# KyanChen/RSPrompter

Hardware: NVIDIA H100
Metric: images/sec (higher is better)
Workload: dtype bf16

## Files before the change

rsprompter_b200/csrc/gemm.h:

```cpp
#pragma once
#include "host_util.h"

namespace rsp {

struct GemmArgs {
  const void* A = nullptr;
  const void* W = nullptr;
  void* out = nullptr;
  const float* bias = nullptr;
  const void* residual = nullptr;
  const int* row_map = nullptr;
  int M = 0, N = 0, K = 0;
  int lda = 0, ldw = 0, ldo = 0, ldr = 0;
  int res_mod = 0;
  int act = 0;
  int out_fp32 = 0;
  int res_fp32 = 1;
  int epi_mode = 0;
  const float* ln_gamma = nullptr;
  const float* ln_beta = nullptr;
  float ln_eps = 1e-6f;
  const int* res_block_map = nullptr;
  int res_block_rows = 0;
  const float* hyper = nullptr;
  float* mask_out = nullptr;
  int grid_h = 0, grid_w = 0;
  int conv_b = 0, conv_h = 0, conv_w = 0, conv_c = 0;
  int m_group_rows = 0, w_group_rows = 0;
};

int gemm_bf16(const GemmArgs& a, cudaStream_t stream);
int gemm_bf16_simt(const GemmArgs& a, cudaStream_t stream);
bool conv3x3_geometry_ok(int B, int H, int W, int C);
int conv3x3_bf16(const GemmArgs& a, cudaStream_t stream);
int gemm_upscale_masks(const GemmArgs& a, int n_out, cudaStream_t stream);

bool gemm_vector_rows(const GemmArgs& a);
int gemm_bf16_v2(const GemmArgs& a, cudaStream_t stream);
int gemm_bf16_v2_gelu_hyper_multi(const GemmArgs& a, int n_out, cudaStream_t stream);

}
```

rsprompter_b200/csrc/gemm_v2.cu:

```cuda
#include "gemm.h"
#include "sm90.cuh"

namespace rsp {

namespace v2 {

constexpr int BM = 128;
constexpr int BK = 64;
constexpr int A_BYTES = BM * BK * 2;
constexpr int STG_ROW = 136;
constexpr int STG_WARP = 32 * STG_ROW;
constexpr int BAR_BYTES = 256;
constexpr int SMEM_MAX = 227 * 1024;

enum { EPI_STD = 0, EPI_LN_ROW = 1, EPI_LN64_GELU = 2, EPI_GELU_HYPER = 3, EPI_GELU_HYPER2 = 4, EPI_GELU_HYPER3 = 5,
       EPI_LN_ROW_T = 6 };

__host__ __device__ constexpr int hyper_outputs(int epi) { return epi == EPI_GELU_HYPER3 ? 3 : epi == EPI_GELU_HYPER2 ? 2 : 1; }

template <int BN, int EPI>
struct Cfg {
  static constexpr bool SPLIT = EPI == EPI_STD;
  static_assert(!SPLIT || BN <= 128, "a 64 x 256 wgmma needs more registers than a 512-thread block has per thread");
  static constexpr int THREADS = SPLIT ? 512 : 384;
  static constexpr int EPI_WARPS = SPLIT ? 4 : 8;
  static constexpr int B_BYTES = BN * BK * 2;
  static constexpr int STAGE_BYTES = A_BYTES + B_BYTES;
  static constexpr int ACC_LD = BN + 4;
  static constexpr int ACC_BYTES = BM * ACC_LD * 4;
  static constexpr int ACC_BUFS = (SPLIT && BN <= 64) ? 2 : 1;
  static constexpr int STG_BYTES = EPI_WARPS * STG_WARP;
  static constexpr int STAGES = SPLIT ? ((BN == 128) ? 4 : (BN == 64) ? 5 : 8) : ((BN == 256) ? 1 : 3);
  static constexpr int SMEM_BYTES = STAGES * STAGE_BYTES + STG_BYTES + ACC_BUFS * ACC_BYTES + BAR_BYTES;
  static_assert(SMEM_BYTES <= SMEM_MAX, "shared memory");
  static_assert(2 * STAGES + 8 + 2 * ACC_BUFS <= BAR_BYTES / 8, "barrier area");
  static constexpr int NHALF = (!SPLIT && BN >= 128 && EPI != EPI_LN_ROW_T) ? 2 : 1;
  static constexpr int COLS_PER_WARP = BN / NHALF;
  static constexpr int REG_PRODUCER = 40;
  static constexpr int REG_MMA = 168;
  static constexpr int REG_EPI = 512 - REG_PRODUCER - 2 * REG_MMA;
  static_assert(REG_EPI >= 128 && REG_EPI % 8 == 0, "the epilogue warpgroup takes registers, never gives them up");
};

struct Dev {
  int M, N, K;
  const float* bias;
  const void* residual;
  void* out;
  const int* row_map;
  const int* res_block_map;
  int res_block_rows;
  int res_mod;
  int ldo, ldr;
  int act;
  int out_fp32;
  int res_fp32;
  int num_n_blocks;
  int num_tiles;
  const float* ln_gamma;
  const float* ln_beta;
  float ln_eps;
  const float* hyper;
  float* mask_out;
  int grid_h, grid_w;
  int conv_kb, conv_h, conv_w;
  int mblk_per_group, w_group_rows;
  int tma_store;
  int tma_res;
  int scalar_rows;
};

__device__ __forceinline__ int num_kblocks(const Dev& p) { return p.conv_kb > 0 ? 9 * p.conv_kb : (p.K + BK - 1) / BK; }

__device__ __forceinline__ int residual_row(const Dev& p, int orow) {
  if (p.res_block_map) {
    const int blk = orow / p.res_block_rows;
    return p.res_block_map[blk] * p.res_block_rows + (orow - blk * p.res_block_rows);
  }
  return p.res_mod > 0 ? (orow % p.res_mod) : orow;
}

__device__ __forceinline__ void add_bias_residual32(const Dev& p, float (&v)[32], int rrow, int col0) {
  if (p.bias) {
    const float4* b4 = reinterpret_cast<const float4*>(p.bias + col0);
#pragma unroll
    for (int i = 0; i < 8; ++i) {
      const float4 b = __ldg(b4 + i);
      v[4 * i + 0] += b.x; v[4 * i + 1] += b.y; v[4 * i + 2] += b.z; v[4 * i + 3] += b.w;
    }
  }
  if (p.residual) {
    if (p.res_fp32) {
      const float4* r4 = reinterpret_cast<const float4*>(
          static_cast<const float*>(p.residual) + static_cast<size_t>(rrow) * p.ldr + col0);
#pragma unroll
      for (int i = 0; i < 8; ++i) {
        const float4 x = r4[i];
        v[4 * i + 0] += x.x; v[4 * i + 1] += x.y; v[4 * i + 2] += x.z; v[4 * i + 3] += x.w;
      }
    } else {
      const uint4* r4 = reinterpret_cast<const uint4*>(
          static_cast<const __nv_bfloat16*>(p.residual) + static_cast<size_t>(rrow) * p.ldr + col0);
#pragma unroll
      for (int i = 0; i < 4; ++i) {
        const uint4 x = r4[i];
        const uint32_t w[4] = {x.x, x.y, x.z, x.w};
#pragma unroll
        for (int j = 0; j < 4; ++j) {
          const __nv_bfloat162 h = *reinterpret_cast<const __nv_bfloat162*>(&w[j]);
          v[8 * i + 2 * j + 0] += __bfloat162float(h.x);
          v[8 * i + 2 * j + 1] += __bfloat162float(h.y);
        }
      }
    }
  }
}

__device__ __forceinline__ void store32(const Dev& p, const float (&v)[32], int orow, int col0) {
  if (p.out_fp32) {
    float4* o4 = reinterpret_cast<float4*>(static_cast<float*>(p.out) + static_cast<size_t>(orow) * p.ldo + col0);
#pragma unroll
    for (int i = 0; i < 8; ++i) o4[i] = make_float4(v[4 * i + 0], v[4 * i + 1], v[4 * i + 2], v[4 * i + 3]);
  } else {
    uint4* o4 = reinterpret_cast<uint4*>(static_cast<__nv_bfloat16*>(p.out) + static_cast<size_t>(orow) * p.ldo + col0);
// ... 576 lines not shown
#pragma unroll
            for (int i = 0; i < 32; ++i) v[i] = fmaxf(v[i], 0.f);
          }
          if (stage_f32) {
            const uint32_t a = stg_s + lane * STG_ROW;
#pragma unroll
            for (int i = 0; i < 16; ++i)
              asm volatile("st.shared.v2.f32 [%0], {%1, %2};" ::"r"(a + i * 8), "f"(v[2 * i]), "f"(v[2 * i + 1])
                           : "memory");
          } else {
            const uint32_t a = stg_s + lane * STG_ROW + c * 64;
#pragma unroll
            for (int i = 0; i < 8; ++i)
              asm volatile("st.shared.v2.b32 [%0], {%1, %2};" ::"r"(a + i * 8),
                           "r"(pack_bf16x2(v[4 * i], v[4 * i + 1])), "r"(pack_bf16x2(v[4 * i + 2], v[4 * i + 3]))
                           : "memory");
          }
        }
        __syncwarp();
        const int col = col_pass + cl * epl;
        if (stage_f32) {
#pragma unroll
          for (int k = 0; k < 16; ++k) {
            const int rr = 2 * k + sub;
            const int orow = get_orow(rr);
            if (orow < 0 || col >= p.N) continue;
            float x0, x1;
            asm volatile("ld.shared.v2.f32 {%0, %1}, [%2];" : "=f"(x0), "=f"(x1) : "r"(stg_s + rr * STG_ROW + cl * 8));
            if (p.residual) {
              if (p.res_fp32 || p.scalar_rows) {
                x0 += resv[k].x; x1 += resv[k].y;
              } else {
                const uint32_t raw = __float_as_uint(resv[k].x);
                x0 += __uint_as_float(raw << 16); x1 += __uint_as_float(raw & 0xffff0000u);
              }
            }
            if (p.scalar_rows) {
              store_at(p, orow, col, x0);
              if (col + 1 < p.N) store_at(p, orow, col + 1, x1);
            } else if (p.out_fp32)
              *reinterpret_cast<float2*>(static_cast<float*>(p.out) + static_cast<size_t>(orow) * p.ldo + col) =
                  make_float2(x0, x1);
            else
              *reinterpret_cast<uint32_t*>(static_cast<__nv_bfloat16*>(p.out) + static_cast<size_t>(orow) * p.ldo +
                                           col) = pack_bf16x2(x0, x1);
          }
        } else {
#pragma unroll 4
          for (int r0 = 0; r0 < 32; r0 += rpi) {
            const int rr = r0 + sub;
            const int orow = get_orow(rr);
            if (orow < 0 || col >= p.N) continue;
            uint32_t w0, w1;
            asm volatile("ld.shared.v2.b32 {%0, %1}, [%2];" : "=r"(w0), "=r"(w1) : "r"(stg_s + rr * STG_ROW + cl * 8));
            *reinterpret_cast<uint2*>(static_cast<__nv_bfloat16*>(p.out) + static_cast<size_t>(orow) * p.ldo + col) =
                make_uint2(w0, w1);
          }
        }
        __syncwarp();
      }
    }
  }
}

template <int BN, int EPI, int OUT>
__device__ __forceinline__ void epilogue_loop(const Dev& p, const CUtensorMap& tma_c, const CUtensorMap& tma_r, int e,
                                              uint32_t acc_base, uint8_t* stg_all, uint64_t* bar_res,
                                              uint64_t* bar_tfull, uint64_t* bar_tempty) {
  using C = Cfg<BN, EPI>;
  uint32_t rphase = 0;
  for (int tile = blockIdx.x; tile < p.num_tiles; tile += gridDim.x) {
    const int m_blk = tile / p.num_n_blocks;
    const int n_blk = tile % p.num_n_blocks;
    const int it = (tile - blockIdx.x) / gridDim.x;
    const int buf = C::ACC_BUFS == 2 ? (it & 1) : 0;
    const uint32_t use = C::ACC_BUFS == 2 ? (it >> 1) : it;
    mbar_wait(smem_u32(&bar_tfull[buf]), use & 1);
    epilogue_tile<BN, EPI, OUT>(p, tma_c, tma_r, m_blk, n_blk, e, 0, acc_base + buf * C::ACC_BYTES, stg_all, bar_res,
                                rphase);
    mbar_arrive(smem_u32(&bar_tempty[buf]));
  }
}

template <int BN, int EPI>
__global__ void __launch_bounds__(Cfg<BN, EPI>::THREADS, 1)
gemm_bf16_wgmma_v2_kernel(const __grid_constant__ CUtensorMap tma_a, const __grid_constant__ CUtensorMap tma_b,
                            const __grid_constant__ CUtensorMap tma_c, const __grid_constant__ CUtensorMap tma_r,
                            const Dev p) {
  using C = Cfg<BN, EPI>;
  constexpr int STAGES = C::STAGES;
  extern __shared__ __align__(1024) uint8_t smem[];
  const uint32_t smem_base = smem_u32(smem);
  uint8_t* stg_all = smem + STAGES * C::STAGE_BYTES;
  const uint32_t acc_base = smem_u32(stg_all + C::STG_BYTES);
  uint64_t* bars = reinterpret_cast<uint64_t*>(stg_all + C::STG_BYTES + C::ACC_BUFS * C::ACC_BYTES);
  uint64_t* bar_full = bars;
  uint64_t* bar_empty = bars + STAGES;
  uint64_t* bar_res = bars + 2 * STAGES;
  uint64_t* bar_tfull = bar_res + 8;
  uint64_t* bar_tempty = bar_tfull + C::ACC_BUFS;

  const int warp = threadIdx.x >> 5;
  const int lane = threadIdx.x & 31;

  if (threadIdx.x == 0) {
    tma_prefetch_desc(&tma_a);
    tma_prefetch_desc(&tma_b);
    for (int s = 0; s < STAGES; ++s) {
      mbar_init(smem_u32(&bar_full[s]), 1);
      mbar_init(smem_u32(&bar_empty[s]), 8);
    }
    for (int s = 0; s < 8; ++s) mbar_init(smem_u32(&bar_res[s]), 1);
    for (int b = 0; b < C::ACC_BUFS; ++b) {
      mbar_init(smem_u32(&bar_tfull[b]), 256);
      mbar_init(smem_u32(&bar_tempty[b]), 32 * C::EPI_WARPS);
    }
    fence_barrier_init();
  }
  __syncthreads();

  if (warp < 4) {
    if constexpr (C::SPLIT) setmaxnreg_dec<C::REG_PRODUCER>();
    if (warp == 0 && lane == 0) {
      const int num_kb = num_kblocks(p);
      int stage = 0;
      uint32_t phase = 0;
      for (int tile = blockIdx.x; tile < p.num_tiles; tile += gridDim.x) {
        const int m_blk = tile / p.num_n_blocks;
        const int n_blk = tile % p.num_n_blocks;
        int cb = 0, cy = 0, cx = 0, tap = 0, ckb = 0;
        const int w_row0 = p.mblk_per_group > 0 ? (m_blk / p.mblk_per_group) * p.w_group_rows : 0;
        if (p.conv_kb > 0) {
          const int hw = p.conv_h * p.conv_w, p0 = m_blk * BM;
          cb = p0 / hw;
          const int rem = p0 - cb * hw;
          cy = rem / p.conv_w;
          cx = rem - cy * p.conv_w;
        }
        for (int kb = 0; kb < num_kb; ++kb) {
          mbar_wait(smem_u32(&bar_empty[stage]), phase ^ 1);
          const uint32_t full = smem_u32(&bar_full[stage]);
          const uint32_t sa = smem_base + stage * C::STAGE_BYTES;
          mbar_expect_tx(full, C::STAGE_BYTES);
          if (p.conv_kb > 0) {
            const int ky = tap / 3, kx = tap - 3 * ky;
            tma_load_4d(sa, &tma_a, full, ckb * BK, cx + kx - 1, cy + ky - 1, cb);
            if (++ckb == p.conv_kb) { ckb = 0; ++tap; }
          } else {
            tma_load_2d(sa, &tma_a, full, kb * BK, m_blk * BM);
          }
          tma_load_2d(sa + A_BYTES, &tma_b, full, kb * BK, n_blk * BN + w_row0);
          if (++stage == STAGES) { stage = 0; phase ^= 1; }
        }
      }
      for (int i = 0; i < STAGES; ++i) {
        mbar_wait(smem_u32(&bar_empty[stage]), phase ^ 1);
        if (++stage == STAGES) { stage = 0; phase ^= 1; }
      }
    }
  } else if (warp < 12) {
    if constexpr (C::SPLIT) setmaxnreg_inc<C::REG_MMA>();
    const int wg = (warp - 4) >> 2;
    const int num_kb = num_kblocks(p);
    int kstage = 0;
    uint32_t kphase = 0;
    if constexpr (C::SPLIT) {
      int it = 0;
      for (int tile = blockIdx.x; tile < p.num_tiles; tile += gridDim.x, ++it) {
        float acc[BN / 2];
        wg_mainloop<BN, STAGES>(acc, smem_base, C::STAGE_BYTES, A_BYTES, num_kb, wg, kstage, kphase, bar_full,
                                bar_empty);
        const int buf = C::ACC_BUFS == 2 ? (it & 1) : 0;
        const uint32_t use = C::ACC_BUFS == 2 ? (it >> 1) : it;
        mbar_wait(smem_u32(&bar_tempty[buf]), (use & 1) ^ 1);
        acc_store<BN>(acc, acc_base + buf * C::ACC_BYTES, C::ACC_LD, wg, threadIdx.x & 127);
        mbar_arrive(smem_u32(&bar_tfull[buf]));
      }
    } else {
      const int e = warp - 4;
      uint32_t rphase = 0;
      for (int tile = blockIdx.x; tile < p.num_tiles; tile += gridDim.x) {
        const int m_blk = tile / p.num_n_blocks;
        const int n_blk = tile % p.num_n_blocks;
        {
          float acc[BN / 2];
          wg_mainloop<BN, STAGES>(acc, smem_base, C::STAGE_BYTES, A_BYTES, num_kb, wg, kstage, kphase, bar_full,
                                  bar_empty);
          named_bar_sync(5, 256);
          acc_store<BN>(acc, acc_base, C::ACC_LD, wg, threadIdx.x & 127);
          named_bar_sync(5, 256);
        }
        if (wg < C::NHALF)
          epilogue_tile<BN, EPI>(p, tma_c, tma_r, m_blk, n_blk, e, wg, acc_base, stg_all, bar_res, rphase);
      }
      if (p.tma_store && lane == 0) bulk_wait0();
    }
  } else if constexpr (C::SPLIT) {
    setmaxnreg_inc<C::REG_EPI>();
    const int e = warp - 12;
    if (p.tma_store) {
      epilogue_loop<BN, EPI, OUT_TMA>(p, tma_c, tma_r, e, acc_base, stg_all, bar_res, bar_tfull, bar_tempty);
      if (lane == 0) bulk_wait0();
    } else {
      epilogue_loop<BN, EPI, OUT_SCATTER>(p, tma_c, tma_r, e, acc_base, stg_all, bar_res, bar_tfull, bar_tempty);
    }
  }
}

template <int BN, int EPI>
static int launch(const GemmArgs& a, cudaStream_t stream) {
  using C = Cfg<BN, EPI>;
  CUtensorMap ta, tb;
  Dev p;
  p.conv_kb = 0; p.conv_h = a.conv_h; p.conv_w = a.conv_w;
  if (a.conv_c > 0) {
    const uint64_t C_ = a.conv_c, W_ = a.conv_w, H_ = a.conv_h, B_ = a.conv_b;
    const uint32_t tw = a.conv_w < BM ? a.conv_w : BM;
    const uint32_t th = (BM / tw) < static_cast<uint32_t>(a.conv_h) ? BM / tw : a.conv_h;
    const uint32_t tb = BM / (tw * th);
    uint64_t dims[4] = {C_, W_, H_, B_};
    uint64_t strides[3] = {C_ * 2, W_ * C_ * 2, H_ * W_ * C_ * 2};
    uint32_t box[4] = {static_cast<uint32_t>(BK), tw, th, tb};
    RSP_TRY(make_tmap_bf16(&ta, a.A, 4, dims, strides, box));
    p.conv_kb = a.conv_c / BK;
  } else {
    RSP_TRY(make_tmap_bf16_2d(&ta, a.A, a.M, a.K, static_cast<uint64_t>(a.lda) * 2, BM, BK));
  }
  const int n_groups = a.m_group_rows > 0 ? (a.M + a.m_group_rows - 1) / a.m_group_rows : 1;
  const uint64_t w_rows = a.m_group_rows > 0 ? static_cast<uint64_t>(n_groups - 1) * a.w_group_rows + a.N : a.N;
  RSP_TRY(make_tmap_bf16_2d(&tb, a.W, w_rows, a.K, static_cast<uint64_t>(a.ldw) * 2, BN, BK));
  CUtensorMap tc = tb, tr = tb;
  p.tma_store = 0;
  p.tma_res = 0;
  p.scalar_rows = EPI == EPI_STD && !gemm_vector_rows(a);
  {
    const uint64_t esz = a.out_fp32 ? 4 : 2;
    bool res_ok = true;
    if (a.residual) {
      res_ok = (a.res_fp32 != 0) == (a.out_fp32 != 0) &&
               (reinterpret_cast<uintptr_t>(a.residual) & 15) == 0 && (static_cast<uint64_t>(a.ldr) * esz) % 16 == 0 &&
               (a.res_block_map ? (a.res_block_rows % 32 == 0 && a.M % 32 == 0) : (a.res_mod == 0 || a.res_mod % 32 == 0));
    }
    if ((EPI == EPI_STD || EPI == EPI_LN_ROW || EPI == EPI_LN64_GELU) && BN >= 64 && res_ok && !a.row_map &&
        !p.scalar_rows && a.out &&
        (reinterpret_cast<uintptr_t>(a.out) & 15) == 0 && (static_cast<uint64_t>(a.ldo) * esz) % 16 == 0) {
      uint64_t dims[2] = {static_cast<uint64_t>(a.N), static_cast<uint64_t>(a.M)};
      uint64_t strides[1] = {static_cast<uint64_t>(a.ldo) * esz};
      uint32_t box[2] = {a.out_fp32 ? 32u : 64u, 32u};
      RSP_TRY(make_tmap(&tc, a.out, 2, dims, strides, box, a.out_fp32));
      p.tma_store = 1;
      if (a.residual) {
        const uint64_t rrows = a.res_block_map ? (1ull << 31) : (a.res_mod > 0 ? a.res_mod : a.M);
        uint64_t rdims[2] = {static_cast<uint64_t>(a.N), rrows};
        uint64_t rstrides[1] = {static_cast<uint64_t>(a.ldr) * esz};
        RSP_TRY(make_tmap(&tr, a.residual, 2, rdims, rstrides, box, a.out_fp32));
        p.tma_res = 1;
      }
    }
  }
  if (EPI == EPI_LN_ROW && !(p.tma_store && p.tma_res)) {
    set_last_error("gemm_v2: fused row LayerNorm needs TMA-eligible bf16 output and residual");
    return RSP_ERR_INVALID;
  }
  p.M = a.M; p.N = a.N; p.K = a.K;
  p.bias = a.bias; p.residual = a.residual; p.out = a.out; p.row_map = a.row_map;
  p.res_block_map = a.res_block_map; p.res_block_rows = a.res_block_rows;
  p.res_mod = a.res_mod; p.ldo = a.ldo; p.ldr = a.ldr; p.act = a.act;
  p.out_fp32 = a.out_fp32; p.res_fp32 = a.res_fp32;
  p.mblk_per_group = a.m_group_rows > 0 ? a.m_group_rows / BM : 0;
  p.w_group_rows = a.w_group_rows;
  p.num_n_blocks = (a.N + BN - 1) / BN;
  p.num_tiles = ((a.M + BM - 1) / BM) * p.num_n_blocks;
  p.ln_gamma = a.ln_gamma; p.ln_beta = a.ln_beta; p.ln_eps = a.ln_eps;
  p.hyper = a.hyper; p.mask_out = a.mask_out; p.grid_h = a.grid_h; p.grid_w = a.grid_w;
  auto kern = gemm_bf16_wgmma_v2_kernel<BN, EPI>;
  static bool attr_set_dev[kMaxDevices] = {};
  bool& attr_set = attr_set_dev[current_device()];
  if (!attr_set) {
    RSP_CHECK_CUDA(cudaFuncSetAttribute(kern, cudaFuncAttributeMaxDynamicSharedMemorySize, C::SMEM_BYTES));
    attr_set = true;
  }
  const int grid = p.num_tiles < num_sms() ? p.num_tiles : num_sms();
  kern<<<grid, C::THREADS, C::SMEM_BYTES, stream>>>(ta, tb, tc, tr, p);
  RSP_CHECK_LAUNCH();
  return RSP_OK;
}

}

bool gemm_vector_rows(const GemmArgs& a) {
  const bool stage_f32 = a.out_fp32 || a.residual;
  const uintptr_t po = reinterpret_cast<uintptr_t>(a.out), pr = reinterpret_cast<uintptr_t>(a.residual);
  if (stage_f32) {
    if (a.N % 2 != 0 || a.ldo % 2 != 0 || (po & (a.out_fp32 ? 7 : 3)) != 0) return false;
  } else {
    if (a.N % 4 != 0 || a.ldo % 4 != 0 || (po & 7) != 0) return false;
  }
  if (a.residual && (a.ldr % 2 != 0 || (pr & (a.res_fp32 ? 7 : 3)) != 0)) return false;
  if (a.bias && (reinterpret_cast<uintptr_t>(a.bias) & 15) != 0) return false;
  return true;
}

static bool ln_row_tma(const GemmArgs& a) {
  return a.N == 256 && !a.out_fp32 && a.residual && !a.res_fp32 && a.bias && a.res_mod == 0 && a.act == 0 &&
         (a.res_block_map ? (a.res_block_rows % 32 == 0 && a.M % 32 == 0) : true);
}

int gemm_bf16_v2(const GemmArgs& a, cudaStream_t stream) {
  if (a.epi_mode == v2::EPI_STD) {
    if (a.N > 64) return v2::launch<128, v2::EPI_STD>(a, stream);
    if (a.N > 32) return v2::launch<64, v2::EPI_STD>(a, stream);
    return v2::launch<32, v2::EPI_STD>(a, stream);
  }
  if (a.epi_mode == v2::EPI_LN_ROW) {
    if (ln_row_tma(a)) return v2::launch<256, v2::EPI_LN_ROW>(a, stream);
    return a.N > 128 ? v2::launch<256, v2::EPI_LN_ROW_T>(a, stream) : v2::launch<128, v2::EPI_LN_ROW_T>(a, stream);
  }
  if (a.epi_mode == v2::EPI_LN64_GELU) return v2::launch<128, v2::EPI_LN64_GELU>(a, stream);
  return v2::launch<128, v2::EPI_GELU_HYPER>(a, stream);
}

int gemm_bf16_v2_gelu_hyper_multi(const GemmArgs& a, int n_out, cudaStream_t stream) {
  switch (n_out) {
    case 1: return v2::launch<128, v2::EPI_GELU_HYPER>(a, stream);
    case 2: return v2::launch<128, v2::EPI_GELU_HYPER2>(a, stream);
    case 3: return v2::launch<128, v2::EPI_GELU_HYPER3>(a, stream);
    default: set_last_error("gemm_v2: %d hypernetwork outputs (1 to 3)", n_out); return RSP_ERR_INVALID;
  }
}

}
```

rsprompter_b200/csrc/selftest.cu:

```cuda
#include <math.h>
#include <stdio.h>
#include <stdlib.h>
#include <string.h>

#include <vector>

#include "gemm.h"
#include "sm90.cuh"

namespace rsp { const char* last_error(); }
using namespace rsp;

#define CK(x)                                                                      \
  do {                                                                             \
    cudaError_t e = (x);                                                           \
    if (e != cudaSuccess) {                                                        \
      printf("CUDA error %s at %s:%d\n", cudaGetErrorString(e), __FILE__, __LINE__); \
      exit(2);                                                                     \
    }                                                                              \
  } while (0)

static uint32_t g_seed = 12345;
static float frand() {
  g_seed = g_seed * 1664525u + 1013904223u;
// ... 64 lines not shown
  a.out = dO1;
  int s = gemm_bf16(a, 0);
  if (s) { printf("[%s] gemm_bf16 failed: %s\n", c.name, last_error()); return 1; }
  cudaError_t e = cudaDeviceSynchronize();
  if (e != cudaSuccess) { printf("[%s] kernel error: %s\n", c.name, cudaGetErrorString(e)); exit(3); }
  a.out = dO2;
  s = gemm_bf16_simt(a, 0);
  if (s) { printf("[%s] simt failed: %s\n", c.name, last_error()); return 1; }
  CK(cudaDeviceSynchronize());
  std::vector<uint8_t> h1(osz), h2(osz);
  CK(cudaMemcpy(h1.data(), dO1, osz, cudaMemcpyDeviceToHost));
  CK(cudaMemcpy(h2.data(), dO2, osz, cudaMemcpyDeviceToHost));
  double maxerr = 0, maxref = 0;
  size_t nbad = 0;
  const size_t n = (size_t)out_rows * N;
  for (size_t i = 0; i < n; ++i) {
    float x, y;
    if (c.out_fp32) { x = ((float*)h1.data())[i]; y = ((float*)h2.data())[i]; }
    else {
      uint32_t ux = (uint32_t)((uint16_t*)h1.data())[i] << 16, uy = (uint32_t)((uint16_t*)h2.data())[i] << 16;
      memcpy(&x, &ux, 4); memcpy(&y, &uy, 4);
    }
    const double d = fabs((double)x - (double)y);
    if (!(d <= 1e-2 * (1.0 + fabs(y)))) ++nbad;
    if (d > maxerr || d != d) maxerr = d;
    if (fabs(y) > maxref) maxref = fabs(y);
  }
  printf("[%s] M=%d N=%d K=%d  max|diff|=%.3e  max|ref|=%.3e  bad=%zu/%zu  %s\n", c.name, M, N, K,
         maxerr, maxref, nbad, n, nbad == 0 ? "PASS" : "FAIL");
  if (nbad) {
    for (int r = 0; r < 4 && r < out_rows; ++r) {
      printf("   row %d:", r);
      for (int j = 0; j < 8 && j < N; ++j) {
        float x, y;
        size_t i = (size_t)r * N + j;
        if (c.out_fp32) { x = ((float*)h1.data())[i]; y = ((float*)h2.data())[i]; }
        else {
          uint32_t ux = (uint32_t)((uint16_t*)h1.data())[i] << 16, uy = (uint32_t)((uint16_t*)h2.data())[i] << 16;
          memcpy(&x, &ux, 4); memcpy(&y, &uy, 4);
        }
        printf(" %.3f/%.3f", x, y);
      }
      printf("\n");
    }
  }
  cudaFree(dA); cudaFree(dW); cudaFree(db); cudaFree(dO1); cudaFree(dO2); cudaFree(dres);
  if (dmap) cudaFree(dmap);
  return nbad ? 1 : 0;
}

static void bench_gemm(int M, int N, int K, int act, int out_fp32, int residual, int res_bf16 = 0, int iters = 20, int res_mod = 0) {
  void *dA, *dW, *dO, *dR = nullptr;
  float* db;
  CK(cudaMalloc(&dA, (size_t)M * K * 2));
  CK(cudaMalloc(&dW, (size_t)N * K * 2));
  CK(cudaMalloc(&dO, (size_t)M * N * 4));
  CK(cudaMalloc(&db, N * 4));
  CK(cudaMemset(dA, 0x11, (size_t)M * K * 2));
  CK(cudaMemset(dW, 0x11, (size_t)N * K * 2));
  CK(cudaMemset(db, 0, N * 4));
  if (residual) { CK(cudaMalloc(&dR, (size_t)M * N * 4)); CK(cudaMemset(dR, 0, (size_t)M * N * 4)); }
  (void)res_bf16;
  GemmArgs a;
  a.A = dA; a.W = dW; a.out = dO; a.bias = db; a.M = M; a.N = N; a.K = K;
  a.lda = K; a.ldw = K; a.ldo = N; a.ldr = N; a.act = act; a.out_fp32 = out_fp32;
  a.residual = dR; a.res_fp32 = res_bf16 ? 0 : 1; a.res_mod = res_mod;
  for (int i = 0; i < 3; ++i) gemm_bf16(a, 0);
  CK(cudaDeviceSynchronize());
  cudaEvent_t e0, e1;
  cudaEventCreate(&e0); cudaEventCreate(&e1);
  cudaEventRecord(e0);
  for (int i = 0; i < iters; ++i) gemm_bf16(a, 0);
  cudaEventRecord(e1);
  CK(cudaDeviceSynchronize());
  float ms;
  cudaEventElapsedTime(&ms, e0, e1);
  ms /= iters;
  const double bytes = (double)M * K * 2 + (double)N * K * 2 + (double)M * N * (out_fp32 ? 4 : 2) +
                       (residual ? (double)M * N * (res_bf16 ? 2 : 4) : 0.0);
  printf("bench gemm M=%d N=%d K=%d act=%d outf32=%d res=%d%s: %.3f ms  %.1f TFLOP/s  %.0f GB/s\n", M, N, K,
         act, out_fp32, residual, res_bf16 ? "(bf16)" : "", ms, 2.0 * M * N * K / ms * 1e-9, bytes / ms * 1e-6);
  cudaFree(dA); cudaFree(dW); cudaFree(dO); cudaFree(db);
  if (dR) cudaFree(dR);
}

int selftest_attention(int bench);


int main(int argc, char** argv) {
  const char* what = argc > 1 ? argv[1] : "all";
  const int bench = argc > 2 && !strcmp(argv[2], "bench");
  int fails = 0;
  cudaDeviceProp prop;
  CK(cudaGetDeviceProperties(&prop, 0));
  printf("device: %s sm_%d%d, %d SMs\n", prop.name, prop.major, prop.minor, prop.multiProcessorCount);
  if (!strcmp(what, "gemm") || !strcmp(what, "all")) {
    const Case cases[] = {
        {"tiny-f32",            128,  128,   64,  0, 0, 0, 1, 1, 0, 0},
        {"k128-f32",            256,  256,  128,  0, 0, 0, 1, 1, 0, 0},
        {"n512-f32",            384,  512,  256,  1, 0, 0, 1, 1, 0, 0},
        {"bn64",                200,   64,  192,  1, 2, 0, 1, 0, 0, 0},
        {"bn32",                200,   32,  192,  1, 2, 0, 1, 0, 0, 0},
        {"ragged-n",            300,   40,  128,  1, 0, 0, 1, 1, 0, 0},
        {"bias-gelu-bf16",     1000,  768,  768,  1, 1, 0, 1, 0, 0, 0},
        {"resid-f32",          1000,  768, 3072,  1, 0, 1, 1, 1, 0, 0},
        {"resid-bf16",          777,  256,  320,  1, 2, 1, 0, 0, 0, 0},
        {"rowmap-resid",       4000, 2304,  768,  1, 0, 1, 1, 1, 1, 0},
        {"posembed-mod",       2048,  768,  768,  1, 0, 1, 1, 1, 0, 512},
        {"multi-tile-per-cta", 40000, 256,  128,  1, 0, 0, 1, 0, 0, 0},
    };
    for (const Case& c : cases) fails += run_case(c);
    if (bench) {
      bench_gemm(39200, 3840, 1280, 0, 0, 0);
      bench_gemm(32768, 1280, 1280, 0, 1, 1);
      bench_gemm(32768, 5120, 1280, 1, 0, 0);
      bench_gemm(32768, 1280, 5120, 0, 1, 1);
      bench_gemm(32768, 768, 3072, 0, 1, 1);
      bench_gemm(8192, 8192, 8192, 0, 0, 0);
    }
  }
  if (!strcmp(what, "gemmprof")) {
    bench_gemm(1 << 20, 256, 128, 0, 1, 1, 1, 3);
    bench_gemm(1 << 20, 128, 256, 0, 0, 0, 0, 3);
    bench_gemm(1 << 20, 256, 128, 0, 0, 0, 0, 3);
    bench_gemm(1 << 20, 128, 256, 0, 0, 1, 0, 3, 4096);
  }
  if (!strcmp(what, "attn") || !strcmp(what, "all")) fails += selftest_attention(bench);
  printf("selftest: %d failing case(s)\n", fails);
  return fails ? 1 : 0;
}
```

rsprompter_b200/csrc/sm90.cuh:

```cuda
#pragma once
#include <cuda.h>
#include <cuda_bf16.h>
#include <cuda_runtime.h>
#include <stdint.h>

namespace rsp {

__device__ __forceinline__ uint32_t smem_u32(const void* p) {
  return static_cast<uint32_t>(__cvta_generic_to_shared(p));
}

__device__ __forceinline__ uint32_t elect_one() {
  uint32_t pred = 0;
  asm volatile(
      "{\n"
      ".reg .b32 rx;\n"
      ".reg .pred px;\n"
      "elect.sync rx|px, 0xffffffff;\n"
      "selp.u32 %0, 1, 0, px;\n"
      "}\n"
      : "=r"(pred));
  return pred;
}

__device__ __forceinline__ void mbar_init(uint32_t bar, uint32_t count) {
  asm volatile("mbarrier.init.shared::cta.b64 [%0], %1;" ::"r"(bar), "r"(count) : "memory");
}
__device__ __forceinline__ void fence_barrier_init() {
  asm volatile("fence.mbarrier_init.release.cluster;" ::: "memory");
}
__device__ __forceinline__ void fence_proxy_async_smem() {
  asm volatile("fence.proxy.async.shared::cta;" ::: "memory");
}
__device__ __forceinline__ void mbar_expect_tx(uint32_t bar, uint32_t bytes) {
  asm volatile("mbarrier.arrive.expect_tx.shared::cta.b64 _, [%0], %1;" ::"r"(bar), "r"(bytes)
               : "memory");
}
__device__ __forceinline__ void mbar_arrive(uint32_t bar) {
  asm volatile("mbarrier.arrive.shared::cta.b64 _, [%0];" ::"r"(bar) : "memory");
}
__device__ __forceinline__ uint32_t mbar_try_wait(uint32_t bar, uint32_t parity) {
  uint32_t ok;
  asm volatile(
      "{\n"
      ".reg .pred p;\n"
      "mbarrier.try_wait.parity.shared::cta.b64 p, [%1], %2;\n"
      "selp.u32 %0, 1, 0, p;\n"
      "}\n"
      : "=r"(ok)
      : "r"(bar), "r"(parity)
      : "memory");
  return ok;
}
__device__ __forceinline__ void mbar_wait(uint32_t bar, uint32_t parity) {
  if (mbar_try_wait(bar, parity)) return;
  long long t0 = clock64();
  uint32_t spins = 0;
  while (!mbar_try_wait(bar, parity)) {
    if ((++spins & 0x3ff) == 0 && clock64() - t0 > (1ll << 31)) __trap();
  }
}

__device__ __forceinline__ void tma_prefetch_desc(const CUtensorMap* m) {
  asm volatile("prefetch.tensormap [%0];" ::"l"(m) : "memory");
}
__device__ __forceinline__ void tma_load_2d(uint32_t dst, const CUtensorMap* m, uint32_t bar,
                                            int c0, int c1) {
  asm volatile(
      "cp.async.bulk.tensor.2d.shared::cluster.global.mbarrier::complete_tx::bytes"
      " [%0], [%1, {%3, %4}], [%2];" ::"r"(dst),
      "l"(m), "r"(bar), "r"(c0), "r"(c1)
      : "memory");
}
__device__ __forceinline__ void tma_load_3d(uint32_t dst, const CUtensorMap* m, uint32_t bar,
                                            int c0, int c1, int c2) {
  asm volatile(
      "cp.async.bulk.tensor.3d.shared::cluster.global.mbarrier::complete_tx::bytes"
      " [%0], [%1, {%3, %4, %5}], [%2];" ::"r"(dst),
      "l"(m), "r"(bar), "r"(c0), "r"(c1), "r"(c2)
      : "memory");
}
__device__ __forceinline__ void tma_load_4d(uint32_t dst, const CUtensorMap* m, uint32_t bar,
                                            int c0, int c1, int c2, int c3) {
  asm volatile(
      "cp.async.bulk.tensor.4d.shared::cluster.global.mbarrier::complete_tx::bytes"
      " [%0], [%1, {%3, %4, %5, %6}], [%2];" ::"r"(dst),
      "l"(m), "r"(bar), "r"(c0), "r"(c1), "r"(c2), "r"(c3)
      : "memory");
}

__device__ __forceinline__ void tma_store_2d(const CUtensorMap* m, uint32_t src, int c0, int c1) {
  asm volatile("cp.async.bulk.tensor.2d.global.shared::cta.bulk_group [%0, {%2, %3}], [%1];" ::"l"(m), "r"(src),
               "r"(c0), "r"(c1)
               : "memory");
}
__device__ __forceinline__ void bulk_commit() { asm volatile("cp.async.bulk.commit_group;" ::: "memory"); }
__device__ __forceinline__ void bulk_wait_read0() { asm volatile("cp.async.bulk.wait_group.read 0;" ::: "memory"); }
__device__ __forceinline__ void bulk_wait0() { asm volatile("cp.async.bulk.wait_group 0;" ::: "memory"); }

__device__ __forceinline__ uint64_t make_gdesc(uint32_t saddr, uint32_t lbo_bytes, uint32_t sbo_bytes) {
  uint64_t d = 0;
  d |= static_cast<uint64_t>((saddr & 0x3ffff) >> 4);
  d |= static_cast<uint64_t>((lbo_bytes >> 4) & 0x3fff) << 16;
  d |= static_cast<uint64_t>((sbo_bytes >> 4) & 0x3fff) << 32;
  d |= 1ull << 62;
  return d;
}

__device__ __forceinline__ uint64_t make_gdesc_sw32(uint32_t saddr, uint32_t lbo_bytes, uint32_t sbo_bytes) {
  uint64_t d = 0;
  d |= static_cast<uint64_t>((saddr & 0x3ffff) >> 4);
  d |= static_cast<uint64_t>((lbo_bytes >> 4) & 0x3fff) << 16;
  d |= static_cast<uint64_t>((sbo_bytes >> 4) & 0x3fff) << 32;
  d |= 3ull << 62;
  return d;
}

__device__ __forceinline__ void wgmma_fence() { asm volatile("wgmma.fence.sync.aligned;" ::: "memory"); }
__device__ __forceinline__ void wgmma_commit() { asm volatile("wgmma.commit_group.sync.aligned;" ::: "memory"); }
template <int N>
__device__ __forceinline__ void wgmma_wait() { asm volatile("wgmma.wait_group.sync.aligned %0;" ::"n"(N) : "memory"); }
template <int R>
__device__ __forceinline__ void acc_fence(float (&d)[R]) {
#pragma unroll
  for (int i = 0; i < R; ++i) asm volatile("" : "+f"(d[i])::"memory");
}

template <int N>
struct Wgmma;
template <> struct Wgmma<32> {
  template <int TB>
  __device__ __forceinline__ static void ss(float (&d)[16], uint64_t a, uint64_t b, uint32_t acc) {
    asm volatile(
        "{\n.reg .pred p;\n"
        "setp.ne.b32 p, %18, 0;\n"
        "wgmma.mma_async.sync.aligned.m64n32k16.f32.bf16.bf16 "
        "{" 
        "%0, %1, %2, %3, %4, %5, %6, %7, %8, %9, %10, %11, %12, %13, %14, %15"
        "}, %16, %17, p, 1, 1, 0, %19;\n}\n"
        : "+f"(d[0]), "+f"(d[1]), "+f"(d[2]), "+f"(d[3]), "+f"(d[4]), "+f"(d[5]), "+f"(d[6]), "+f"(d[7]),
          "+f"(d[8]), "+f"(d[9]), "+f"(d[10]), "+f"(d[11]), "+f"(d[12]), "+f"(d[13]), "+f"(d[14]), "+f"(d[15])
        : "l"(a), "l"(b), "r"(acc), "n"(TB));
  }
};
template <> struct Wgmma<64> {
  template <int TB>
  __device__ __forceinline__ static void ss(float (&d)[32], uint64_t a, uint64_t b, uint32_t acc) {
    asm volatile(
        "{\n.reg .pred p;\n"
        "setp.ne.b32 p, %34, 0;\n"
        "wgmma.mma_async.sync.aligned.m64n64k16.f32.bf16.bf16 "
        "{" 
        "%0, %1, %2, %3, %4, %5, %6, %7, %8, %9, %10, %11, %12, %13, %14, %15, "
        "%16, %17, %18, %19, %20, %21, %22, %23, %24, %25, %26, %27, %28, %29, %30, %31"
        "}, %32, %33, p, 1, 1, 0, %35;\n}\n"
        : "+f"(d[0]), "+f"(d[1]), "+f"(d[2]), "+f"(d[3]), "+f"(d[4]), "+f"(d[5]), "+f"(d[6]), "+f"(d[7]),
          "+f"(d[8]), "+f"(d[9]), "+f"(d[10]), "+f"(d[11]), "+f"(d[12]), "+f"(d[13]), "+f"(d[14]), "+f"(d[15]),
          "+f"(d[16]), "+f"(d[17]), "+f"(d[18]), "+f"(d[19]), "+f"(d[20]), "+f"(d[21]), "+f"(d[22]), "+f"(d[23]),
          "+f"(d[24]), "+f"(d[25]), "+f"(d[26]), "+f"(d[27]), "+f"(d[28]), "+f"(d[29]), "+f"(d[30]), "+f"(d[31])
        : "l"(a), "l"(b), "r"(acc), "n"(TB));
  }
};
template <> struct Wgmma<128> {
  template <int TB>
  __device__ __forceinline__ static void ss(float (&d)[64], uint64_t a, uint64_t b, uint32_t acc) {
    asm volatile(
        "{\n.reg .pred p;\n"
        "setp.ne.b32 p, %66, 0;\n"
        "wgmma.mma_async.sync.aligned.m64n128k16.f32.bf16.bf16 "
        "{" 
        "%0, %1, %2, %3, %4, %5, %6, %7, %8, %9, %10, %11, %12, %13, %14, %15, "
        "%16, %17, %18, %19, %20, %21, %22, %23, %24, %25, %26, %27, %28, %29, %30, %31, "
        "%32, %33, %34, %35, %36, %37, %38, %39, %40, %41, %42, %43, %44, %45, %46, %47, "
        "%48, %49, %50, %51, %52, %53, %54, %55, %56, %57, %58, %59, %60, %61, %62, %63"
        "}, %64, %65, p, 1, 1, 0, %67;\n}\n"
        : "+f"(d[0]), "+f"(d[1]), "+f"(d[2]), "+f"(d[3]), "+f"(d[4]), "+f"(d[5]), "+f"(d[6]), "+f"(d[7]),
          "+f"(d[8]), "+f"(d[9]), "+f"(d[10]), "+f"(d[11]), "+f"(d[12]), "+f"(d[13]), "+f"(d[14]), "+f"(d[15]),
          "+f"(d[16]), "+f"(d[17]), "+f"(d[18]), "+f"(d[19]), "+f"(d[20]), "+f"(d[21]), "+f"(d[22]), "+f"(d[23]),
          "+f"(d[24]), "+f"(d[25]), "+f"(d[26]), "+f"(d[27]), "+f"(d[28]), "+f"(d[29]), "+f"(d[30]), "+f"(d[31]),
          "+f"(d[32]), "+f"(d[33]), "+f"(d[34]), "+f"(d[35]), "+f"(d[36]), "+f"(d[37]), "+f"(d[38]), "+f"(d[39]),
// ... 211 lines not shown
```

Before: 61.16.

## Add 128x256 wide GEMM schedule with register epilogue for large plain GEMMs

Adds a new EPI_STD_WIDE kernel variant that uses 128x256 tiles. The two MMA warpgroups hold 232 registers each and run the epilogue straight from registers, writing swizzled bf16 slabs to shared memory and storing them with double-buffered TMA stores. This drops the separate epilogue warpgroup and the fp32 shared-memory accumulator staging. The variant is selected automatically for plain bias/activation GEMMs with N divisible by 256, K >= 1024 and enough tiles. This raises per-tile arithmetic intensity but serialises the epilogue with the mainloop for each tile, so there is no overlap. A/B benchmarks and a correctness case are added to the selftest.

New measurement: 63.07 (median of 6 runs). 1.03x the previous value.

```diff
diff --git a/rsprompter_b200/csrc/gemm.h b/rsprompter_b200/csrc/gemm.h
--- a/rsprompter_b200/csrc/gemm.h
+++ b/rsprompter_b200/csrc/gemm.h
@@ -37,6 +37,7 @@
 
 bool gemm_vector_rows(const GemmArgs& a);
 int gemm_bf16_v2(const GemmArgs& a, cudaStream_t stream);
+int gemm_bf16_v2_std(const GemmArgs& a, bool wide, cudaStream_t stream);
 int gemm_bf16_v2_gelu_hyper_multi(const GemmArgs& a, int n_out, cudaStream_t stream);
 
 }
diff --git a/rsprompter_b200/csrc/gemm_v2.cu b/rsprompter_b200/csrc/gemm_v2.cu
--- a/rsprompter_b200/csrc/gemm_v2.cu
+++ b/rsprompter_b200/csrc/gemm_v2.cu
@@ -14,7 +14,7 @@
 constexpr int SMEM_MAX = 227 * 1024;
 
 enum { EPI_STD = 0, EPI_LN_ROW = 1, EPI_LN64_GELU = 2, EPI_GELU_HYPER = 3, EPI_GELU_HYPER2 = 4, EPI_GELU_HYPER3 = 5,
-       EPI_LN_ROW_T = 6 };
+       EPI_LN_ROW_T = 6, EPI_STD_WIDE = 7 };
 
 __host__ __device__ constexpr int hyper_outputs(int epi) { return epi == EPI_GELU_HYPER3 ? 3 : epi == EPI_GELU_HYPER2 ? 2 : 1; }
 
@@ -22,24 +22,28 @@
 struct Cfg {
   static constexpr bool SPLIT = EPI == EPI_STD;
   static_assert(!SPLIT || BN <= 128, "a 64 x 256 wgmma needs more registers than a 512-thread block has per thread");
+  static constexpr bool WIDE = EPI == EPI_STD_WIDE;
+  static_assert(!WIDE || BN == 256, "the register epilogue is written for the 64 x 256 fragment");
   static constexpr int THREADS = SPLIT ? 512 : 384;
   static constexpr int EPI_WARPS = SPLIT ? 4 : 8;
   static constexpr int B_BYTES = BN * BK * 2;
   static constexpr int STAGE_BYTES = A_BYTES + B_BYTES;
   static constexpr int ACC_LD = BN + 4;
   static constexpr int ACC_BYTES = BM * ACC_LD * 4;
-  static constexpr int ACC_BUFS = (SPLIT && BN <= 64) ? 2 : 1;
+  static constexpr int ACC_BUFS = WIDE ? 0 : (SPLIT && BN <= 64) ? 2 : 1;
   static constexpr int STG_BYTES = EPI_WARPS * STG_WARP;
-  static constexpr int STAGES = SPLIT ? ((BN == 128) ? 4 : (BN == 64) ? 5 : 8) : ((BN == 256) ? 1 : 3);
+  static constexpr int STAGES =
+      WIDE ? 4 : SPLIT ? ((BN == 128) ? 4 : (BN == 64) ? 5 : 8) : ((BN == 256) ? 1 : 3);
   static constexpr int SMEM_BYTES = STAGES * STAGE_BYTES + STG_BYTES + ACC_BUFS * ACC_BYTES + BAR_BYTES;
   static_assert(SMEM_BYTES <= SMEM_MAX, "shared memory");
   static_assert(2 * STAGES + 8 + 2 * ACC_BUFS <= BAR_BYTES / 8, "barrier area");
   static constexpr int NHALF = (!SPLIT && BN >= 128 && EPI != EPI_LN_ROW_T) ? 2 : 1;
   static constexpr int COLS_PER_WARP = BN / NHALF;
   static constexpr int REG_PRODUCER = 40;
-  static constexpr int REG_MMA = 168;
-  static constexpr int REG_EPI = 512 - REG_PRODUCER - 2 * REG_MMA;
-  static_assert(REG_EPI >= 128 && REG_EPI % 8 == 0, "the epilogue warpgroup takes registers, never gives them up");
+  static constexpr int REG_MMA = WIDE ? 232 : 168;
+  static_assert(!WIDE || REG_PRODUCER + 2 * REG_MMA <= 3 * 168, "wide schedule register budget");
+  static constexpr int REG_EPI = SPLIT ? 512 - REG_PRODUCER - 2 * REG_MMA : 0;
+  static_assert(!SPLIT || (REG_EPI >= 128 && REG_EPI % 8 == 0), "the epilogue warpgroup takes registers, never gives them up");
 };
 
 struct Dev {
@@ -782,6 +786,44 @@
   }
 }
 
+__device__ __forceinline__ void epilogue_wide(const Dev& p, const CUtensorMap& tma_c, const float (&acc)[128],
+                                              int m_blk, int n_blk, int wg, int e, uint8_t* stg_all) {
+  const int lane = threadIdx.x & 31;
+  const int r = lane >> 2;
+  const int row0 = m_blk * BM + wg * 64 + (e & 3) * 16;
+  const uint32_t slab = smem_u32(stg_all) + e * 4096;
+  const float* bias = p.bias;
+  const int act = p.act;
+#pragma unroll
+  for (int s = 0; s < 4; ++s) {
+    const int col0 = n_blk * 256 + s * 64;
+    const uint32_t half = slab + (s & 1) * 2048;
+    if (lane == 0) bulk_wait_read1();
+    __syncwarp();
+#pragma unroll
+    for (int c = 0; c < 8; ++c) {
+      float v[4] = {acc[32 * s + 4 * c], acc[32 * s + 4 * c + 1], acc[32 * s + 4 * c + 2], acc[32 * s + 4 * c + 3]};
+      if (bias) {
+        const float2 b = __ldg(reinterpret_cast<const float2*>(bias + col0 + 8 * c + 2 * (lane & 3)));
+        v[0] += b.x; v[1] += b.y; v[2] += b.x; v[3] += b.y;
+      }
+      if (act == 1) {
+#pragma unroll
+        for (int i = 0; i < 4; ++i) v[i] = gelu_fast(v[i]);
+      } else if (act == 2) {
+#pragma unroll
+        for (int i = 0; i < 4; ++i) v[i] = fmaxf(v[i], 0.f);
+      }
+      const uint32_t a = half + r * 128 + ((c ^ r) << 4) + 4 * (lane & 3);
+      asm volatile("st.shared.b32 [%0], %1;" ::"r"(a), "r"(pack_bf16x2(v[0], v[1])) : "memory");
+      asm volatile("st.shared.b32 [%0], %1;" ::"r"(a + 8 * 128), "r"(pack_bf16x2(v[2], v[3])) : "memory");
+    }
+    fence_proxy_async_smem();
+    __syncwarp();
+    if (lane == 0) { tma_store_2d(&tma_c, half, col0, row0); bulk_commit(); }
+  }
+}
+
 template <int BN, int EPI>
 __global__ void __launch_bounds__(Cfg<BN, EPI>::THREADS, 1)
 gemm_bf16_wgmma_v2_kernel(const __grid_constant__ CUtensorMap tma_a, const __grid_constant__ CUtensorMap tma_b,
@@ -820,7 +862,7 @@
   __syncthreads();
 
   if (warp < 4) {
-    if constexpr (C::SPLIT) setmaxnreg_dec<C::REG_PRODUCER>();
+    if constexpr (C::SPLIT || C::WIDE) setmaxnreg_dec<C::REG_PRODUCER>();
     if (warp == 0 && lane == 0) {
       const int num_kb = num_kblocks(p);
       int stage = 0;
@@ -859,12 +901,20 @@
       }
     }
   } else if (warp < 12) {
-    if constexpr (C::SPLIT) setmaxnreg_inc<C::REG_MMA>();
+    if constexpr (C::SPLIT || C::WIDE) setmaxnreg_inc<C::REG_MMA>();
     const int wg = (warp - 4) >> 2;
     const int num_kb = num_kblocks(p);
     int kstage = 0;
     uint32_t kphase = 0;
-    if constexpr (C::SPLIT) {
+    if constexpr (C::WIDE) {
+      for (int tile = blockIdx.x; tile < p.num_tiles; tile += gridDim.x) {
+        float acc[BN / 2];
+        wg_mainloop<BN, STAGES>(acc, smem_base, C::STAGE_BYTES, A_BYTES, num_kb, wg, kstage, kphase, bar_full,
+                                bar_empty);
+        epilogue_wide(p, tma_c, acc, tile / p.num_n_blocks, tile % p.num_n_blocks, wg, warp - 4, stg_all);
+      }
+      if (lane == 0) bulk_wait0();
+    } else if constexpr (C::SPLIT) {
       int it = 0;
       for (int tile = blockIdx.x; tile < p.num_tiles; tile += gridDim.x, ++it) {
         float acc[BN / 2];
@@ -941,12 +991,12 @@
                (reinterpret_cast<uintptr_t>(a.residual) & 15) == 0 && (static_cast<uint64_t>(a.ldr) * esz) % 16 == 0 &&
                (a.res_block_map ? (a.res_block_rows % 32 == 0 && a.M % 32 == 0) : (a.res_mod == 0 || a.res_mod % 32 == 0));
     }
-    if ((EPI == EPI_STD || EPI == EPI_LN_ROW || EPI == EPI_LN64_GELU) && BN >= 64 && res_ok && !a.row_map &&
-        !p.scalar_rows && a.out &&
+    if ((EPI == EPI_STD || EPI == EPI_STD_WIDE || EPI == EPI_LN_ROW || EPI == EPI_LN64_GELU) && BN >= 64 && res_ok &&
+        !a.row_map && !p.scalar_rows && a.out &&
         (reinterpret_cast<uintptr_t>(a.out) & 15) == 0 && (static_cast<uint64_t>(a.ldo) * esz) % 16 == 0) {
       uint64_t dims[2] = {static_cast<uint64_t>(a.N), static_cast<uint64_t>(a.M)};
       uint64_t strides[1] = {static_cast<uint64_t>(a.ldo) * esz};
-      uint32_t box[2] = {a.out_fp32 ? 32u : 64u, 32u};
+      uint32_t box[2] = {a.out_fp32 ? 32u : 64u, C::WIDE ? 16u : 32u};
       RSP_TRY(make_tmap(&tc, a.out, 2, dims, strides, box, a.out_fp32));
       p.tma_store = 1;
       if (a.residual) {
@@ -960,6 +1010,10 @@
   }
   if (EPI == EPI_LN_ROW && !(p.tma_store && p.tma_res)) {
     set_last_error("gemm_v2: fused row LayerNorm needs TMA-eligible bf16 output and residual");
+    return RSP_ERR_INVALID;
+  }
+  if (C::WIDE && !(p.tma_store && !a.residual && !a.out_fp32 && a.N % BN == 0 && a.conv_c == 0 && a.m_group_rows == 0)) {
+    set_last_error("gemm_v2: the wide schedule needs a plain GEMM with TMA-eligible bf16 output, no residual, N %% 256 == 0");
     return RSP_ERR_INVALID;
   }
   p.M = a.M; p.N = a.N; p.K = a.K;
@@ -1006,11 +1060,24 @@
          (a.res_block_map ? (a.res_block_rows % 32 == 0 && a.M % 32 == 0) : true);
 }
 
+static bool std_wide_shape(const GemmArgs& a) {
+  return a.epi_mode == v2::EPI_STD && !a.residual && !a.row_map && !a.out_fp32 && a.conv_c == 0 &&
+         a.m_group_rows == 0 && a.N % 256 == 0 && a.K % 64 == 0 && gemm_vector_rows(a) && a.out &&
+         (reinterpret_cast<uintptr_t>(a.out) & 15) == 0 && a.ldo % 8 == 0;
+}
+
+int gemm_bf16_v2_std(const GemmArgs& a, bool wide, cudaStream_t stream) {
+  if (wide) return v2::launch<256, v2::EPI_STD_WIDE>(a, stream);
+  if (a.N > 64) return v2::launch<128, v2::EPI_STD>(a, stream);
+  if (a.N > 32) return v2::launch<64, v2::EPI_STD>(a, stream);
+  return v2::launch<32, v2::EPI_STD>(a, stream);
+}
+
 int gemm_bf16_v2(const GemmArgs& a, cudaStream_t stream) {
   if (a.epi_mode == v2::EPI_STD) {
-    if (a.N > 64) return v2::launch<128, v2::EPI_STD>(a, stream);
-    if (a.N > 32) return v2::launch<64, v2::EPI_STD>(a, stream);
-    return v2::launch<32, v2::EPI_STD>(a, stream);
+    const long long wide_tiles = static_cast<long long>((a.M + v2::BM - 1) / v2::BM) * (a.N / 256);
+    const bool wide = std_wide_shape(a) && a.K >= 1024 && wide_tiles >= 16ll * num_sms();
+    return gemm_bf16_v2_std(a, wide, stream);
   }
   if (a.epi_mode == v2::EPI_LN_ROW) {
     if (ln_row_tma(a)) return v2::launch<256, v2::EPI_LN_ROW>(a, stream);
diff --git a/rsprompter_b200/csrc/selftest.cu b/rsprompter_b200/csrc/selftest.cu
--- a/rsprompter_b200/csrc/selftest.cu
+++ b/rsprompter_b200/csrc/selftest.cu
@@ -170,6 +170,65 @@
          act, out_fp32, residual, res_bf16 ? "(bf16)" : "", ms, 2.0 * M * N * K / ms * 1e-9, bytes / ms * 1e-6);
   cudaFree(dA); cudaFree(dW); cudaFree(dO); cudaFree(db);
   if (dR) cudaFree(dR);
+}
+
+static int bench_gemm_ab(const char* name, int M, int N, int K, int act, int rounds = 5, int iters = 10) {
+  std::vector<uint16_t> hA((size_t)M * K), hW((size_t)N * K);
+  for (auto& x : hA) x = f2bf(frand());
+  for (auto& x : hW) x = f2bf(frand() * 0.25f);
+  std::vector<float> hb(N);
+  for (auto& x : hb) x = frand();
+  void *dA, *dW, *dO[2];
+  float* db;
+  const size_t osz = (size_t)M * N * 2;
+  CK(cudaMalloc(&dA, hA.size() * 2));
+  CK(cudaMalloc(&dW, hW.size() * 2));
+  CK(cudaMalloc(&db, N * 4));
+  CK(cudaMalloc(&dO[0], osz));
+  CK(cudaMalloc(&dO[1], osz));
+  CK(cudaMemcpy(dA, hA.data(), hA.size() * 2, cudaMemcpyHostToDevice));
+  CK(cudaMemcpy(dW, hW.data(), hW.size() * 2, cudaMemcpyHostToDevice));
+  CK(cudaMemcpy(db, hb.data(), N * 4, cudaMemcpyHostToDevice));
+  CK(cudaMemset(dO[0], 0xff, osz));
+  CK(cudaMemset(dO[1], 0x7f, osz));
+  GemmArgs a;
+  a.A = dA; a.W = dW; a.bias = db; a.M = M; a.N = N; a.K = K;
+  a.lda = K; a.ldw = K; a.ldo = N; a.act = act;
+  for (int w = 0; w < 2; ++w) {
+    a.out = dO[w];
+    for (int i = 0; i < 3; ++i)
+      if (gemm_bf16_v2_std(a, w == 1, 0)) { printf("[%s] launch failed: %s\n", name, last_error()); exit(3); }
+  }
+  CK(cudaDeviceSynchronize());
+  cudaEvent_t e0, e1;
+  cudaEventCreate(&e0); cudaEventCreate(&e1);
+  float ms[2] = {0.f, 0.f};
+  for (int r = 0; r < rounds; ++r) {
+    for (int w = 0; w < 2; ++w) {
+      a.out = dO[w];
+      cudaEventRecord(e0);
+      for (int i = 0; i < iters; ++i) gemm_bf16_v2_std(a, w == 1, 0);
+      cudaEventRecord(e1);
+      CK(cudaEventSynchronize(e1));
+      float t;
+      cudaEventElapsedTime(&t, e0, e1);
+      ms[w] += t;
+    }
+  }
+  std::vector<uint8_t> h0(osz), h1(osz);
+  CK(cudaMemcpy(h0.data(), dO[0], osz, cudaMemcpyDeviceToHost));
+  CK(cudaMemcpy(h1.data(), dO[1], osz, cudaMemcpyDeviceToHost));
+  size_t ndiff = 0;
+  for (size_t i = 0; i < osz; i += 2) ndiff += memcmp(&h0[i], &h1[i], 2) != 0;
+  const double flop = 2.0 * M * N * K;
+  const double t128 = ms[0] / (rounds * iters), t256 = ms[1] / (rounds * iters);
+  printf("ab gemm %-10s M=%d N=%d K=%d act=%d: 128x128 %.3f ms %.1f TFLOP/s | 128x256 %.3f ms %.1f TFLOP/s | "
+         "speed-up %.3f | outputs %s (%zu of %zu differ)\n",
+         name, M, N, K, act, t128, flop / t128 * 1e-9, t256, flop / t256 * 1e-9, t128 / t256,
+         ndiff ? "DIFFER" : "identical", ndiff, osz / 2);
+  cudaEventDestroy(e0); cudaEventDestroy(e1);
+  cudaFree(dA); cudaFree(dW); cudaFree(db); cudaFree(dO[0]); cudaFree(dO[1]);
+  return ndiff ? 1 : 0;
 }
 
 int selftest_attention(int bench);
@@ -196,6 +255,7 @@
         {"rowmap-resid",       4000, 2304,  768,  1, 0, 1, 1, 1, 1, 0},
         {"posembed-mod",       2048,  768,  768,  1, 0, 1, 1, 1, 0, 512},
         {"multi-tile-per-cta", 40000, 256,  128,  1, 0, 0, 1, 0, 0, 0},
+        {"wide-bias-gelu",    65000, 1280, 1024,  1, 1, 0, 1, 0, 0, 0},
     };
     for (const Case& c : cases) fails += run_case(c);
     if (bench) {
@@ -205,6 +265,17 @@
       bench_gemm(32768, 1280, 5120, 0, 1, 1);
       bench_gemm(32768, 768, 3072, 0, 1, 1);
       bench_gemm(8192, 8192, 8192, 0, 0, 0);
+      fails += bench_gemm_ab("vith-qkv", 39200, 3840, 1280, 0);
+      fails += bench_gemm_ab("vith-qkv", 32768, 3840, 1280, 0);
+      fails += bench_gemm_ab("vith-lin1", 32768, 5120, 1280, 1);
+      fails += bench_gemm_ab("vitb-qkv", 39200, 2304, 768, 0);
+      fails += bench_gemm_ab("vitb-qkv", 32768, 2304, 768, 0);
+      fails += bench_gemm_ab("vitb-lin1", 32768, 3072, 768, 1);
+      for (int m : {1024, 2048, 4096, 8192}) {
+        fails += bench_gemm_ab("vith-qkv", m, 3840, 1280, 0);
+        fails += bench_gemm_ab("vith-lin1", m, 5120, 1280, 1);
+      }
+      for (int k : {256, 512}) fails += bench_gemm_ab("k-sweep", 32768, 1280, k, 0);
     }
   }
   if (!strcmp(what, "gemmprof")) {
diff --git a/rsprompter_b200/csrc/sm90.cuh b/rsprompter_b200/csrc/sm90.cuh
--- a/rsprompter_b200/csrc/sm90.cuh
+++ b/rsprompter_b200/csrc/sm90.cuh
@@ -96,6 +96,7 @@
 }
 __device__ __forceinline__ void bulk_commit() { asm volatile("cp.async.bulk.commit_group;" ::: "memory"); }
 __device__ __forceinline__ void bulk_wait_read0() { asm volatile("cp.async.bulk.wait_group.read 0;" ::: "memory"); }
+__device__ __forceinline__ void bulk_wait_read1() { asm volatile("cp.async.bulk.wait_group.read 1;" ::: "memory"); }
 __device__ __forceinline__ void bulk_wait0() { asm volatile("cp.async.bulk.wait_group 0;" ::: "memory"); }
 
 __device__ __forceinline__ uint64_t make_gdesc(uint32_t saddr, uint32_t lbo_bytes, uint32_t sbo_bytes) {
```
